# dmlc/difacto

Hardware: AMD Instinct MI355X
Metric: examples/sec (FM SGD worker step, Criteo-shape, V_dim=64) (higher is better)
Workload: dtype f32

## Files before the change

difacto_amd/csrc/dfh_api.hip:

```cpp
#include <algorithm>
#include <chrono>
#include <cstring>
#include <mutex>
#include <new>
#include <thread>

#include <hip/hip_ext.h>
#include <rocprim/rocprim.hpp>

#include "dfh_kernels.hip"
#include "dfh_localize.hip"
#include "dfh_update.hip"
#include "dfh_riders.hip"

using namespace dfh;

namespace dfh {
static thread_local std::string g_err;
void set_error(const std::string& msg) { g_err = msg; }
}

struct dfh_ctx {
  int device = 0;
  hipStream_t stream = nullptr;
// ... 2424 lines not shown
  }
  DFH_ARG(total == nrows, "dfh_batch_gather_rows: the segments must hold nrows rows");
  DFH_HIP(hipSetDevice(b->ctx->device));
  phase_begin(b);
  rc = prep_begin(b);
  if (rc) return rc;
  hipStream_t s = prep_of(b);
  b->d_raw = b->o_raw; b->d_offset = b->o_offset; b->d_value = b->o_value; b->d_label = b->o_label;
  const size_t o_off = 0, o_lab = (b->max_rows + 1) * 4, o_idx = ((o_lab + b->max_rows * 4 + 255) & ~(size_t)255),
               o_val = o_idx + b->max_nnz * 8, stage_total = o_val + b->max_nnz * 4;
  (void)stage_total;
  rc = ensure_stage(b, o_idx + (b->max_rows + 1) * 4);
  if (rc) return rc;
  if (b->staged_pending) {
    if (hipEventQuery(b->ev_staged) != hipSuccess) DFH_HIP(hipEventSynchronize(b->ev_staged));
    b->staged_pending = false;
  }
  memcpy(b->h_stage + o_off, off32.data(), (nrows + 1) * 4);
  memcpy(b->h_stage + o_lab, label, nrows * 4);
  uint32_t* h_rows = reinterpret_cast<uint32_t*>(b->h_stage + o_idx);
  size_t at = 0;
  for (int g = 0; g < nseg; ++g) {
    for (size_t i = 0; i < seg_rows[g]; ++i) {
      DFH_ARG(rows[g][i] < bufs[g]->nrows, "dfh_batch_gather_rows: row number beyond the buffer");
      h_rows[at + i] = rows[g][i];
    }
    at += seg_rows[g];
  }
  uint32_t* d_rows = b->d_pos;
  DFH_HIP(hipMemcpyAsync(b->d_offset, b->h_stage + o_off, (nrows + 1) * 4, hipMemcpyHostToDevice, s));
  DFH_HIP(hipMemcpyAsync(b->d_label, b->h_stage + o_lab, nrows * 4, hipMemcpyHostToDevice, s));
  DFH_HIP(hipMemcpyAsync(d_rows, h_rows, nrows * 4, hipMemcpyHostToDevice, s));
  DFH_HIP(hipEventRecord(b->ev_staged, s));
  b->staged_pending = true;
  at = 0;
  for (int g = 0; g < nseg; ++g) {
    dfh_rowbuf* rb = bufs[g];
    if (seg_rows[g] == 0) continue;
    DFH_HIP(hipStreamWaitEvent(s, rb->ev_loaded, 0));
    const unsigned blocks = (unsigned)std::min<size_t>((seg_rows[g] + 3) / 4, 4096);
    hipLaunchKernelGGL(k_gather_rows, dim3(blocks), dim3(256), 0, s, rb->d_off, rb->d_idx, rb->has_value ? rb->d_val : (const float*)nullptr,
                       d_rows + at, (uint32_t)seg_rows[g], b->d_offset + at, b->d_raw, any_value ? b->d_value : (float*)nullptr);
    {
      std::lock_guard<std::mutex> lk(rb->mu);
      dfh_rowbuf::Used* u = nullptr;
      for (auto& x : rb->used)
        if (x.stream == s) u = &x;
      if (!u) {
        hipEvent_t ev = nullptr;
        DFH_HIP(hipEventCreateWithFlags(&ev, hipEventDisableTiming));
        rb->used.push_back({s, ev, false});
        u = &rb->used.back();
      }
      DFH_HIP(hipEventRecord(u->ev, s));
      u->pending = true;
    }
    at += seg_rows[g];
  }
  DFH_HIP(hipGetLastError());
  b->nrows = nrows;
  b->nnz = nnz;
  b->has_value = any_value;
  b->has_cnt = false;
  b->localized = false;
  b->looked_up = nullptr;
  return DFH_OK;
}

namespace {
__global__ void __launch_bounds__(256) k_gather_rows_staged(const uint32_t* __restrict__ src_off, const uint64_t* __restrict__ src_idx,
                                                            const float* __restrict__ src_val, const uint32_t* __restrict__ h_rows,
                                                            const uint32_t* __restrict__ h_off, const float* __restrict__ h_lab, uint32_t n,
                                                            uint32_t* __restrict__ dst_off, float* __restrict__ dst_lab,
                                                            uint64_t* __restrict__ dst_idx, float* __restrict__ dst_val, int write_end) {
  constexpr uint32_t GR = 32;
  __shared__ uint32_t s_lo[GR], s_len[GR], s_d0[GR];
  const uint32_t lane = threadIdx.x & 63u, w = threadIdx.x >> 6;
  for (uint32_t q0 = blockIdx.x * GR; q0 < n; q0 += gridDim.x * GR) {
    const uint32_t m = min(GR, n - q0);
    __syncthreads();
    if (threadIdx.x < m) {
      const uint32_t q = q0 + threadIdx.x;
      const uint32_t r = h_rows[q], o = h_off[q];
      const uint32_t lo = src_off[r];
      s_lo[threadIdx.x] = lo;
      s_len[threadIdx.x] = src_off[r + 1] - lo;
      s_d0[threadIdx.x] = o;
      dst_off[q] = o;
      dst_lab[q] = h_lab[q];
    }
    if (threadIdx.x == 255 && write_end && q0 + m == n) dst_off[n] = h_off[n];
    __syncthreads();
    for (uint32_t t = w; t < m; t += 4u) {
      const uint32_t lo = s_lo[t], len = s_len[t], d0 = s_d0[t];
      for (uint32_t j = lane; j < len; j += 64u) {
        dst_idx[d0 + j] = src_idx[lo + j];
        if (dst_val) dst_val[d0 + j] = src_val ? src_val[lo + j] : 1.0f;
      }
    }
  }
}
}

namespace {
int gather_queued(dfh_batch* b, hipStream_t s) {
  for (const auto& g : b->gsegs) {
    dfh_rowbuf* rb = g.rb;
    std::lock_guard<std::mutex> lk(rb->mu);
    dfh_rowbuf::Used* u = nullptr;
    for (auto& x : rb->used)
      if (x.stream == s) u = &x;
    if (!u) {
      hipEvent_t ev = nullptr;
      DFH_HIP(hipEventCreateWithFlags(&ev, hipEventDisableTiming));
      rb->used.push_back({s, ev, false});
      u = &rb->used.back();
    }
    DFH_HIP(hipEventRecord(u->ev, s));
    u->pending = true;
  }
  DFH_HIP(hipEventRecord(b->ev_staged, s));
  b->staged_pending = true;
  b->gather_pending = false;
  return DFH_OK;
}
int gather_alone(dfh_batch* b, hipStream_t s) {
  for (const auto& g : b->gsegs) {
    dfh_rowbuf* rb = g.rb;
    const unsigned blocks = (unsigned)std::min<size_t>((g.n + 31) / 32, 2048);
    hipLaunchKernelGGL(k_gather_rows_staged, dim3(blocks), dim3(256), 0, s, rb->d_off, rb->d_idx,
                       rb->has_value ? rb->d_val : (const float*)nullptr, b->g_rows + g.at, b->g_off + g.at, b->g_lab + g.at, (uint32_t)g.n,
                       b->d_offset + g.at, b->d_label + g.at, b->d_raw, b->gather_any_value ? b->d_value : (float*)nullptr,
                       g.at + g.n == b->nrows ? 1 : 0);
  }
  DFH_HIP(hipGetLastError());
  return gather_queued(b, s);
}
}

namespace {
void launch_loc_stage(dfh_batch* b, int stage, hipStream_t s, dfh_table* probe = nullptr) {
  const LocView& v = b->loc_v;
  switch (stage) {
    case RID_COUNT:
      if (b->loc_big) hipLaunchKernelGGL(k_loc_count<LOC_BIG_BUCKETS>, dim3(v.ntiles), dim3(LOC_TILE_THREADS), 0, s, v);
      else if (b->loc_fuse_gather) hipLaunchKernelGGL(k_loc_count_gather<LOC_MAX_BUCKETS>, dim3(v.ntiles), dim3(LOC_TILE_THREADS), 0, s, v, b->gsrc);
      else hipLaunchKernelGGL(k_loc_count<LOC_MAX_BUCKETS>, dim3(v.ntiles), dim3(LOC_TILE_THREADS), 0, s, v);
      break;
    case RID_SCATTER:
      if (b->loc_big) hipLaunchKernelGGL(k_loc_scatter<LOC_BIG_BUCKETS>, dim3(v.ntiles), dim3(LOC_TILE_THREADS), 0, s, v);
      else hipLaunchKernelGGL(k_loc_scatter<LOC_MAX_BUCKETS>, dim3(v.ntiles), dim3(LOC_TILE_THREADS), 0, s, v);
      break;
    case RID_SORT:
      hipLaunchKernelGGL(k_loc_sort, dim3(b->loc_gsort), dim3(LOC_SORT_THREADS), 0, s, v);
      break;
    default:
      if (probe) hipLaunchKernelGGL(k_loc_emit<true>, dim3(b->loc_gsort), dim3(LOC_EMIT_THREADS), 0, s, v, b->loc_o, probe->v, b->d_urow);
      else hipLaunchKernelGGL(k_loc_emit<false>, dim3(b->loc_gsort), dim3(LOC_EMIT_THREADS), 0, s, v, b->loc_o, TableView{}, (uint32_t*)nullptr);
      break;
  }
}

void pend_remove(dfh_ctx* c, dfh_batch* b) {
  auto it = std::find(c->pend.begin(), c->pend.end(), b);
  if (it != c->pend.end()) c->pend.erase(it);
}

int flush_pending(dfh_batch* b) {
  dfh_ctx* c = b->ctx;
  if (b->pend_stage >= RID_STAGES) return DFH_OK;
  {
    TimeScope ts(c, DFH_K_LOCALIZE);
    for (int st = b->pend_stage; st < RID_STAGES; ++st) launch_loc_stage(b, st, c->stream);
  }
  b->pend_stage = RID_STAGES;
  pend_remove(c, b);
  DFH_HIP(hipGetLastError());
  return DFH_OK;
}

void collect_riders(dfh_ctx* c, int slot, bool can_ride, uint32_t main_groups, RiderSet* rs) {
  rs->n = 0;
  rs->ngroups = 0;
  rs->period = 1;
  rs->start = 0;
  rs->first[0] = 0;
  if (!c->single_queue || c->pend.empty()) return;
  for (size_t i = 0; i < c->pend.size(); ++i) {
    dfh_batch* p = c->pend[i];
    while (p->pend_stage < RID_STAGES && c->rider_slot[p->pend_stage] == slot) {
      const int st = p->pend_stage;
      if (c->rider_alone[st] || !can_ride || rs->n == MAX_RIDERS) {
        TimeScope ts(c, DFH_K_LOCALIZE);
        launch_loc_stage(p, st, c->stream);
        ++p->pend_stage;
        continue;
      }
      Rider& r = rs->r[rs->n];
      r.v = p->loc_v;
      r.o = p->loc_o;
      r.kind = (uint32_t)st;
      r.nblk = (st == RID_COUNT || st == RID_SCATTER) ? (uint32_t)p->loc_v.ntiles : p->loc_gsort;
      rs->first[rs->n + 1] = rs->first[rs->n] + ((r.nblk + 7u) & ~7u);
      ++rs->n;
      ++p->pend_stage;
      break;
    }
  }
  for (uint32_t j = 1; j < rs->n; ++j) {
    if (rs->r[j].kind == RID_EMIT && rs->r[0].kind != RID_EMIT) {
      std::swap(rs->r[0], rs->r[j]);
      uint32_t at = 0;
      for (uint32_t q = 0; q < rs->n; ++q) {
        rs->first[q] = at;
        at += (rs->r[q].nblk + 7u) & ~7u;
      }
      rs->first[rs->n] = at;
      break;
    }
  }
  c->pend.erase(std::remove_if(c->pend.begin(), c->pend.end(), [](dfh_batch* p) { return p->pend_stage >= RID_STAGES; }), c->pend.end());
  rs->ngroups = rs->first[rs->n] / 8u;
  for (uint32_t q = rs->n + 1; q <= (uint32_t)MAX_RIDERS; ++q) rs->first[q] = rs->first[rs->n];
  if (rs->ngroups) {
    rs->start = (uint32_t)((uint64_t)main_groups * (uint64_t)c->rider_start[slot] / 100u);
    const uint32_t left = main_groups - rs->start;
    uint32_t per = (uint32_t)std::max(1, c->rider_period[slot]);
    if (rs->ngroups > 1) per = std::min(per, (left + rs->ngroups - 1u) / (rs->ngroups - 1u));
    rs->period = std::max(1u, per);
  }
}

int localize_impl(dfh_batch* b, uint64_t max_index, dfh_table* probe) {
  dfh_ctx* c = b->ctx;
  DFH_HIP(hipSetDevice(c->device));
  const uint32_t N = (uint32_t)b->nnz;
  if (probe && N) {
    if (int rcr = table_reserve(probe, N)) return rcr;
  }
  {
    int rc = prep_begin(b);
    if (rc) return rc;
  }
  hipStream_t s = prep_of(b);
  b->looked_up = nullptr;
  if (b->pend_stage < RID_STAGES) {
    int rc = flush_pending(b);
    if (rc) return rc;
  }
  if (N == 0) {
    if (b->gather_pending) {
      int rcg = gather_alone(b, s);
      if (rcg) return rcg;
    }
    DFH_HIP(hipMemsetAsync(b->d_U, 0, 64 * sizeof(uint32_t), s));
    DFH_HIP(hipMemsetAsync(b->d_col_ptr, 0, 4, s));
    b->seg_nb = 0;
    b->localized = true;
    return prep_end(b);
  }
  const int g = grid_for_threads(N, c);
  TimeScope* tsp = new TimeScope(c, DFH_K_LOCALIZE, s);
  int P = 0;
  bool cold = true;
  if (b->spl_P > 0 && N / (uint32_t)b->spl_P >= (uint32_t)LOC_MIN_AVG && N / (uint32_t)b->spl_P <= (uint32_t)LOC_MAX_AVG) {
    P = b->spl_P;
    cold = false;
  } else {
#ifndef DFH_LOC_SMALL_AVG
#define DFH_LOC_SMALL_AVG 192
#endif
    const size_t avg_bucket = N <= 65536u ? (size_t)DFH_LOC_SMALL_AVG : (size_t)LOC_AVG_BUCKET;
    const size_t P_want = (N + avg_bucket - 1) / avg_bucket;
    if (P_want <= (size_t)LOC_MAX_BUCKETS) P = (int)std::max<size_t>(1, P_want);
    else if (N / LOC_MAX_BUCKETS <= (uint32_t)LOC_MAX_AVG) P = LOC_MAX_BUCKETS;
    else if (P_want <= (size_t)LOC_BIG_BUCKETS) P = (int)P_want;
    else if (N / LOC_BIG_BUCKETS <= (uint32_t)LOC_MAX_AVG) P = LOC_BIG_BUCKETS;
  }
  b->loc_fuse_gather = b->gather_pending && b->gather_fusable && !cold && P > 0 && P <= LOC_MAX_BUCKETS && !b->force_radix &&
                       !c->single_queue && !getenv("DFH_GATHER_ALONE");
  if (b->gather_pending && !b->loc_fuse_gather) {
    int rcg = gather_alone(b, s);
    if (rcg) return rcg;
  }
  if (P > 0 && !b->force_radix) {
    LocView& v = b->loc_v;
    v.raw = b->d_raw;
    v.n = N;
    v.max_index = max_index;
    v.P = P;
    const bool big = P > LOC_MAX_BUCKETS;
    v.bstride = big ? LOC_BIG_BUCKETS : LOC_MAX_BUCKETS;
    v.ntiles = (int)((N + LOC_TILE - 1) / LOC_TILE);
    v.force_global = b->force_sort_fallback ? 1 : 0;
    v.tb = N > 1 ? std::min(16, __builtin_clz(N - 1)) : 16;
    v.nrows = (uint32_t)b->nrows;
    v.offset = b->d_offset;
    v.rowid = b->d_pos;
    v.smp_key = b->d_smp_key;
    v.smp_pos = b->d_smp_pos;
    v.smp_rank = b->d_smp_rank;
    v.spl_key = b->d_spl_key;
    v.spl_pos = b->d_spl_pos;
    v.packed = b->d_packed;
    v.run_off = b->d_run_off;
    v.btotal = b->d_btotal;
    v.bstart = b->d_bstart;
// ... 653 lines not shown
```

difacto_amd/csrc/dfh_localize.hip:

```cpp
#ifndef DFH_LOCALIZE_HIP_
#define DFH_LOCALIZE_HIP_
#include "dfh_internal.h"

namespace dfh {

constexpr int LOC_OVERSAMPLE = 8;
constexpr int LOC_MAX_BUCKETS = 1024;
constexpr int LOC_BIG_BUCKETS = 4096;
constexpr int LOC_AVG_BUCKET = 384;
constexpr int LOC_MIN_AVG = 48;
constexpr int LOC_MAX_AVG = 700;
constexpr int LOC_LDS_CAP = 1024;
#ifndef DFH_LOC_TILE
#define DFH_LOC_TILE 2048
#endif
#ifndef DFH_LOC_TILE_THREADS
#define DFH_LOC_TILE_THREADS 1024
#endif
constexpr int LOC_TILE = DFH_LOC_TILE;
constexpr int LOC_TILE_THREADS = DFH_LOC_TILE_THREADS;
constexpr int LOC_PER_THREAD = LOC_TILE / LOC_TILE_THREADS;
constexpr int LOC_SORT_THREADS = 256;
constexpr int LOC_EMIT_THREADS = 256;

struct LocView {
  const uint64_t* raw;
  uint32_t n;
  uint64_t max_index;
  int P;
  int bstride;
  int ntiles;
  int force_global;
  int tb;
  uint32_t nrows;
  const uint32_t* offset;
  const uint32_t* rowid;
  uint64_t* smp_key;
  uint32_t* smp_pos;
  uint32_t* smp_rank;
  uint64_t* spl_key;
  uint32_t* spl_pos;
  uint32_t* packed;
  uint32_t* run_off;
  uint32_t* btotal;
  uint32_t* bstart;
  uint64_t* bkeys;
  uint32_t* bpos;
  uint64_t* skeys;
  uint32_t* spos;
  uint64_t* first_key;
  uint64_t* last_key;
  uint32_t* nheads;
  uint32_t* lh;
  uint32_t* split_n;
};

struct SegListsOut {
  uint2* mid;
  SegEnt* mid_ent;
  uint2* hot;
  SegEnt* hot_ent;
  uint2* few;
  SegEnt* few_ent;
};

__device__ __forceinline__ uint64_t make_key(uint64_t id, uint64_t max_index) {
  const uint64_t m = (max_index == ~0ULL) ? (id == ~0ULL ? 0ULL : id) : id % max_index;
  return reverse_bytes(m);
}

constexpr int LOC_XCDS = 8;

__device__ __forceinline__ bool comp_less(uint64_t ka, uint32_t pa, uint64_t kb, uint32_t pb) {
  return ka < kb || (ka == kb && pa < pb);
}

template <int NWAVES>
__device__ __forceinline__ uint32_t block_exclusive_scan(uint32_t val, uint32_t* wsum , uint32_t* total) {
  uint32_t s = val;
#pragma unroll
  for (int o = 1; o < 64; o <<= 1) {
    const uint32_t y = __shfl_up(s, o, 64);
    if ((int)(threadIdx.x & 63) >= o) s += y;
  }
  __syncthreads();
  if ((threadIdx.x & 63) == 63) wsum[threadIdx.x >> 6] = s;
  __syncthreads();
  uint32_t woff = 0, tot = 0;
#pragma unroll
  for (int w = 0; w < NWAVES; ++w) {
    const uint32_t x = wsum[w];
    if (w < (int)(threadIdx.x >> 6)) woff += x;
    tot += x;
  }
  if (total) *total = tot;
  return woff + s - val;
}

template <int NWAVES>
__device__ __forceinline__ uint32_t block_exclusive_max(uint32_t val, uint32_t* wmax , uint32_t* total) {
  uint32_t s = val;
#pragma unroll
  for (int o = 1; o < 64; o <<= 1) {
    const uint32_t y = __shfl_up(s, o, 64);
    if ((int)(threadIdx.x & 63) >= o) s = max(s, y);
  }
  __syncthreads();
  if ((threadIdx.x & 63) == 63) wmax[threadIdx.x >> 6] = s;
  __syncthreads();
  uint32_t before = 0, tot = 0;
#pragma unroll
  for (int w = 0; w < NWAVES; ++w) {
    const uint32_t x = wmax[w];
    if (w < (int)(threadIdx.x >> 6)) before = max(before, x);
    tot = max(tot, x);
  }
  if (total) *total = tot;
  uint32_t prev = __shfl_up(s, 1, 64);
  if ((threadIdx.x & 63) == 0) prev = 0;
  return max(before, prev);
}

__device__ __forceinline__ uint32_t ss_sample_pos(uint32_t t, uint32_t stride, uint32_t n) {
  const uint32_t j = (uint32_t)(splitmix64(t) >> 33) % stride;
  return min(t * stride + j, n - 1);
}

__global__ void __launch_bounds__(256) k_ss_sample(LocView v) {
  const uint32_t S = (uint32_t)v.P * LOC_OVERSAMPLE;
  const uint32_t stride = max(1u, v.n / S);
  for (uint32_t t = blockIdx.x * blockDim.x + threadIdx.x; t < S; t += gridDim.x * blockDim.x) {
    const uint32_t i = ss_sample_pos(t, stride, v.n);
    v.smp_key[t] = make_key(v.raw[i], v.max_index);
    v.smp_pos[t] = i << v.tb;
    v.smp_rank[t] = 0;
  }
}

__global__ void __launch_bounds__(256) k_ss_rank(LocView v) {
  __shared__ uint64_t ck[256];
  __shared__ uint32_t cp[256];
  const uint32_t S = (uint32_t)v.P * LOC_OVERSAMPLE;
  const uint32_t ntile = (S + 255) / 256;
  const uint32_t ti = blockIdx.x / ntile, tj = blockIdx.x % ntile;
  const uint32_t col = tj * 256 + threadIdx.x;
  ck[threadIdx.x] = col < S ? v.smp_key[col] : ~0ULL;
  cp[threadIdx.x] = col < S ? v.smp_pos[col] : ~0u;
  const uint32_t row = ti * 256 + threadIdx.x;
  const uint64_t mk = row < S ? v.smp_key[row] : 0;
  const uint32_t mp = row < S ? v.smp_pos[row] : 0;
  __syncthreads();
  const uint32_t lim = min(256u, S - tj * 256);
  uint32_t rank = 0;
#pragma unroll 8
  for (uint32_t j = 0; j < lim; ++j) {
    const bool less = comp_less(ck[j], cp[j], mk, mp) || (ck[j] == mk && cp[j] == mp && tj * 256 + j < row);
    rank += less ? 1u : 0u;
  }
  if (row < S && rank) atomicAdd(&v.smp_rank[row], rank);
}

__global__ void __launch_bounds__(256) k_loc_splitters(LocView v) {
  const uint32_t S = (uint32_t)v.P * LOC_OVERSAMPLE;
  for (uint32_t t = blockIdx.x * blockDim.x + threadIdx.x; t < S; t += gridDim.x * blockDim.x) {
    const uint32_t r = v.smp_rank[t];
    if (r > 0 && r % LOC_OVERSAMPLE == 0) {
      v.spl_key[r / LOC_OVERSAMPLE - 1] = v.smp_key[t];
      v.spl_pos[r / LOC_OVERSAMPLE - 1] = v.smp_pos[t];
    }
  }
}

constexpr int LOC_GATHER_ROWS = 1024;
constexpr int LOC_GATHER_SEGS = 4;
struct GatherSrc {
  int nseg;
  uint32_t seg_row0[LOC_GATHER_SEGS + 1];
  const uint32_t* src_off[LOC_GATHER_SEGS];
  const uint64_t* src_idx[LOC_GATHER_SEGS];
  const float* src_val[LOC_GATHER_SEGS];
  const uint32_t* h_rows;
  const uint32_t* h_off;
  const float* h_lab;
  const uint32_t* h_tile_row;
  uint64_t* dst_raw;
  float* dst_val;
  uint32_t* dst_off;
  float* dst_lab;
};
constexpr size_t loc_gather_smem() { return (size_t)(LOC_GATHER_ROWS + 1) * 4 + 4 + (size_t)LOC_GATHER_ROWS * 8; }
template <typename T>
__device__ __forceinline__ T loc_sel(const T (&a)[LOC_GATHER_SEGS], uint32_t sg) {
  T r = a[0];
#pragma unroll
  for (int x = 1; x < LOC_GATHER_SEGS; ++x) r = sg == (uint32_t)x ? a[x] : r;
  return r;
}

template <int MAXB>
constexpr size_t loc_count_smem() { return (size_t)MAXB * 16; }
template <int MAXB, int THREADS>
constexpr size_t loc_scatter_smem() { return (size_t)MAXB * 4 + (THREADS / 64) * 4; }
constexpr size_t loc_sort_smem() { return (size_t)LOC_LDS_CAP * 24 + 2 * (LOC_SORT_THREADS / 64) * 4; }
constexpr size_t loc_emit_smem() { return (2 * (LOC_EMIT_THREADS / 64) + 4) * 4; }

template <int MAXB, int THREADS, bool GATHER = false>
__device__ __forceinline__ void loc_count_block(const LocView& v, const uint32_t bid, const uint32_t nblk, char* smem,
                                                const GatherSrc* gp = nullptr) {
  constexpr int PER = LOC_TILE / THREADS;
  static_assert(PER * THREADS == LOC_TILE, "a tile is a whole number of elements per thread");
  uint64_t* sk = reinterpret_cast<uint64_t*>(smem);
  uint32_t* sp = reinterpret_cast<uint32_t*>(smem + (size_t)MAXB * 8);
  uint32_t* hist = sp + MAXB;
  const int P = v.P;
  for (int b = threadIdx.x; b < P; b += THREADS) {
    hist[b] = 0;
    sk[b] = b < P - 1 ? v.spl_key[b] : ~0ULL;
    sp[b] = b < P - 1 ? v.spl_pos[b] : ~0u;
  }
  const uint32_t base = bid * LOC_TILE;
  if (bid == 0 && threadIdx.x == 0 && v.split_n) *v.split_n = 0u;
  uint64_t key[PER];
  if (GATHER) {
    const GatherSrc& g = *gp;
    uint32_t* roff = reinterpret_cast<uint32_t*>(smem + loc_count_smem<MAXB>());
    uint64_t* rsrc = reinterpret_cast<uint64_t*>(roff + LOC_GATHER_ROWS + 2);
    const uint32_t row0 = g.h_tile_row[bid], row1 = g.h_tile_row[bid + 1];
    const uint32_t nr = min(row1, v.nrows - 1u) - row0 + 1u;
    for (uint32_t q = threadIdx.x; q <= nr; q += THREADS) roff[q] = g.h_off[row0 + q];
    for (uint32_t q = threadIdx.x; q < nr; q += THREADS) {
      const uint32_t r = row0 + q;
      uint32_t sg = 0;
#pragma unroll
      for (int x = 1; x < LOC_GATHER_SEGS; ++x) sg += (x < g.nseg && r >= g.seg_row0[x]) ? 1u : 0u;
      rsrc[q] = ((uint64_t)loc_sel(g.src_off, sg)[g.h_rows[r]] << 2) | sg;
    }
    __syncthreads();
#pragma unroll
    for (int e = 0; e < PER; ++e) {
      const uint32_t i = base + e * THREADS + threadIdx.x;
      key[e] = ~0ULL;
      if (i < v.n) {
        uint32_t lo = 0, hi = nr - 1u;
        while (lo < hi) {
          const uint32_t mid = (lo + hi + 1u) >> 1;
          if (roff[mid] <= i) lo = mid; else hi = mid - 1u;
        }
        const uint64_t sw = rsrc[lo];
        const uint32_t sg = (uint32_t)(sw & 3u);
        const size_t at = (size_t)(sw >> 2) + (i - roff[lo]);
        const uint64_t id = loc_sel(g.src_idx, sg)[at];
        g.dst_raw[i] = id;
        if (g.dst_val) {
          const float* sv = loc_sel(g.src_val, sg);
          g.dst_val[i] = sv ? sv[at] : 1.0f;
        }
        key[e] = make_key(id, v.max_index);
      }
    }
  } else {
#pragma unroll
    for (int e = 0; e < PER; ++e) {
      const uint32_t i = base + e * THREADS + threadIdx.x;
      key[e] = i < v.n ? make_key(v.raw[i], v.max_index) : ~0ULL;
    }
  }
  {
    uint32_t* __restrict__ rowid = const_cast<uint32_t*>(v.rowid);
    const uint32_t* __restrict__ offset = GATHER ? gp->h_off : v.offset;
    const uint32_t rpb = (v.nrows + nblk - 1) / nblk;
    const uint32_t r0 = bid * rpb, r1 = min(v.nrows, r0 + rpb);
    for (uint32_t r = r0 + threadIdx.x; r < r1; r += THREADS) {
      const uint32_t b0 = offset[r], e = offset[r + 1];
      if (GATHER) {
        gp->dst_off[r] = b0;
        gp->dst_lab[r] = gp->h_lab[r];
        if (r + 1 == v.nrows) gp->dst_off[r + 1] = e;
      }
      for (uint32_t j = b0; j < e; ++j) rowid[j] = r;
    }
  }
  __syncthreads();
  int lo[PER], hi[PER];
#pragma unroll
  for (int e = 0; e < PER; ++e) { lo[e] = 0; hi[e] = P - 1; }
  for (int step = P; step > 1; step = (step + 1) >> 1) {
#pragma unroll
    for (int e = 0; e < PER; ++e) {
      if (lo[e] < hi[e]) {
        const uint32_t i = base + e * THREADS + threadIdx.x;
        const int mid = (lo[e] + hi[e]) >> 1;
        if (comp_less(key[e], i << v.tb, sk[mid], sp[mid])) hi[e] = mid; else lo[e] = mid + 1;
      }
    }
  }
#pragma unroll
  for (int e = 0; e < PER; ++e) {
    const uint32_t i = base + e * THREADS + threadIdx.x;
    if (i < v.n) {
      const uint32_t r = atomicAdd(&hist[lo[e]], 1u);
      v.packed[i] = ((uint32_t)lo[e] << 16) | r;
    }
  }
  __syncthreads();
  for (int b = threadIdx.x; b < P; b += THREADS) {
    const uint32_t h = hist[b];
    v.run_off[bid * P + b] = h ? atomicAdd(&v.btotal[(bid & (LOC_XCDS - 1)) * MAXB + b], h) : 0u;
  }
}

template <int MAXB>
__global__ void __launch_bounds__(LOC_TILE_THREADS) k_loc_count(LocView v) {
  __shared__ __attribute__((aligned(16))) char smem[loc_count_smem<MAXB>()];
  loc_count_block<MAXB, LOC_TILE_THREADS>(v, blockIdx.x, gridDim.x, smem);
}
template <int MAXB>
__global__ void __launch_bounds__(LOC_TILE_THREADS) k_loc_count_gather(LocView v, GatherSrc g) {
  __shared__ __attribute__((aligned(16))) char smem[loc_count_smem<MAXB>() + loc_gather_smem()];
  loc_count_block<MAXB, LOC_TILE_THREADS, true>(v, blockIdx.x, gridDim.x, smem, &g);
}


template <int MAXB, int THREADS>
__device__ __forceinline__ void loc_scatter_block(const LocView& v, const uint32_t bid, char* smem) {
  constexpr int PER = LOC_TILE / THREADS;
  constexpr int LOC_BPT = MAXB / THREADS;
  static_assert(LOC_BPT * THREADS == MAXB, "the scan of the bucket totals gives every thread the same number of buckets");
  uint32_t* off = reinterpret_cast<uint32_t*>(smem);
  uint32_t* wsum = off + MAXB;
  const int P = v.P;
  const uint32_t xcd = bid & (LOC_XCDS - 1);
  const uint32_t base = bid * LOC_TILE;
  uint64_t raw[PER];
  uint32_t pk[PER], rw[PER];
#pragma unroll
  for (int e = 0; e < PER; ++e) {
    const uint32_t i = min(base + e * THREADS + threadIdx.x, v.n - 1);
    raw[e] = v.raw[i];
    pk[e] = v.packed[i];
    rw[e] = v.rowid[i];
  }
  const int b0 = threadIdx.x * LOC_BPT;
  uint32_t tt[LOC_BPT], ro[LOC_BPT];
  uint32_t sum = 0;
#pragma unroll
  for (int q = 0; q < LOC_BPT; ++q) {
    const int bb = min(b0 + q, P - 1);
    const uint32_t in = b0 + q < P ? 1u : 0u;
    tt[q] = 0;
    ro[q] = v.run_off[bid * P + bb];
#pragma unroll
    for (int x = 0; x < LOC_XCDS; ++x) {
      const uint32_t h = v.btotal[x * MAXB + bb];
      tt[q] += h;
      ro[q] += (x < (int)xcd ? 1u : 0u) * h;
    }
    tt[q] *= in;
    ro[q] *= in;
    sum += tt[q];
  }
  uint32_t total;
  uint32_t ex = block_exclusive_scan<THREADS / 64>(sum, wsum, &total);
#pragma unroll
  for (int q = 0; q < LOC_BPT; ++q) {
    if (b0 + q < P) {
      off[b0 + q] = ex + ro[q];
      if (bid == 0) v.bstart[b0 + q] = ex;
    }
    ex += tt[q];
  }
  if (bid == 0 && threadIdx.x == 0) v.bstart[P] = total;
  __syncthreads();
#pragma unroll
  for (int e = 0; e < PER; ++e) {
    const uint32_t i = base + e * THREADS + threadIdx.x;
    if (i < v.n) {
      const uint32_t dst = off[pk[e] >> 16] + (pk[e] & 0xFFFFu);
      v.bkeys[dst] = make_key(raw[e], v.max_index);
      v.bpos[dst] = (i << v.tb) | (rw[e] & ((1u << v.tb) - 1u));
    }
  }
}

template <int MAXB>
__global__ void __launch_bounds__(LOC_TILE_THREADS) k_loc_scatter(LocView v) {
  __shared__ __attribute__((aligned(16))) char smem[loc_scatter_smem<MAXB, LOC_TILE_THREADS>()];
  loc_scatter_block<MAXB, LOC_TILE_THREADS>(v, blockIdx.x, smem);
}

__device__ __forceinline__ bool loc_sort_bucket(const LocView& v, uint32_t beg, uint32_t n, uint64_t* ak, uint32_t* ap,
                                                uint64_t* bk, uint32_t* bp, const uint64_t** sk_out, const uint32_t** sp_out) {
  const uint64_t* gk = v.bkeys + beg;
  const uint32_t* gp = v.bpos + beg;
  const bool in_lds = n <= LOC_LDS_CAP && !v.force_global;
  uint64_t* sk = bk;
  uint32_t* sp = bp;
  if (in_lds) {
    const uint32_t lane = threadIdx.x & 63;
    for (uint32_t c0 = (threadIdx.x >> 6) * 64; c0 < n; c0 += LOC_SORT_THREADS) {
      const uint32_t idx = c0 + lane;
      const bool valid = idx < n;
      const uint64_t mk = valid ? gk[idx] : ~0ULL;
      const uint32_t mp = valid ? gp[idx] : ~0u;
      const int klo = (int)(uint32_t)mk, khi = (int)(uint32_t)(mk >> 32);
      uint32_t rank = 0;
#pragma unroll 8
      for (int j = 0; j < 64; ++j) {
        const uint64_t ok = ((uint64_t)(uint32_t)__builtin_amdgcn_readlane(khi, j) << 32) | (uint32_t)__builtin_amdgcn_readlane(klo, j);
        const uint32_t op = (uint32_t)__builtin_amdgcn_readlane((int)mp, j);
        rank += comp_less(ok, op, mk, mp) ? 1u : 0u;
      }
      if (valid) {
        bk[c0 + rank] = mk;
        bp[c0 + rank] = mp;
      }
    }
    __syncthreads();
    constexpr int E = LOC_LDS_CAP / LOC_SORT_THREADS;
    static_assert(E * LOC_SORT_THREADS == LOC_LDS_CAP && LOC_SORT_THREADS % 64 == 0, "a thread carries E elements of a full bucket");
    uint64_t* dk = ak;
    uint32_t* dp = ap;
    uint32_t sh = 6;
    for (uint32_t L = 64; L < n; L <<= 1, ++sh) {
      uint64_t mk[E];
      uint32_t mp[E], cnt[E], sb[E], len[E];
#pragma unroll
      for (int e = 0; e < E; ++e) {
        const uint32_t idx = threadIdx.x + e * LOC_SORT_THREADS;
        const bool valid = idx < n;
        len[e] = 0;
        cnt[e] = 0;
        if (e * LOC_SORT_THREADS >= n) continue;
        mk[e] = valid ? sk[idx] : 0ULL;
        mp[e] = valid ? sp[idx] : 0u;
        const uint32_t sib = ((idx >> sh) ^ 1u) << sh;
        sb[e] = min(sib, n);
        len[e] = valid ? min(sib + L, n) - sb[e] : 0u;
        cnt[e] = 0;
      }
      for (uint32_t step = L; step; step >>= 1) {
        uint64_t ok[E];
        uint32_t op[E];
#pragma unroll
        for (int e = 0; e < E; ++e) {
          if (e * LOC_SORT_THREADS >= n) continue;
          const uint32_t t = cnt[e] + step;
          const uint32_t at = t <= len[e] ? sb[e] + t - 1u : 0u;
          ok[e] = sk[at];
          op[e] = sp[at];
        }
#pragma unroll
        for (int e = 0; e < E; ++e) {
          if (e * LOC_SORT_THREADS >= n) continue;
          const uint32_t t = cnt[e] + step;
          if (t <= len[e] && comp_less(ok[e], op[e], mk[e], mp[e])) cnt[e] = t;
        }
      }
#pragma unroll
      for (int e = 0; e < E; ++e) {
        const uint32_t idx = threadIdx.x + e * LOC_SORT_THREADS;
        if (idx < n) {
          const uint32_t r = idx >> sh;
          const uint32_t dst = ((r & ~1u) << sh) + (idx - (r << sh)) + cnt[e];
          dk[dst] = mk[e];
          dp[dst] = mp[e];
        }
      }
      __syncthreads();
      uint64_t* tk = sk; sk = dk; dk = tk;
      uint32_t* tp = sp; sp = dp; dp = tp;
    }
    *sk_out = sk;
    *sp_out = sp;
  } else {
    uint64_t* xk = v.bkeys + beg;
    uint32_t* xp = v.bpos + beg;
    uint64_t* yk = v.skeys + beg;
    uint32_t* yp = v.spos + beg;
    const uint32_t lane = threadIdx.x & 63;
    for (uint32_t c0 = (threadIdx.x >> 6) * 64; c0 < n; c0 += LOC_SORT_THREADS) {
      const uint32_t idx = c0 + lane;
      const bool valid = idx < n;
      const uint64_t mk = valid ? xk[idx] : ~0ULL;
      const uint32_t mp = valid ? xp[idx] : ~0u;
      const uint32_t lim = min(64u, n - c0);
      uint32_t rank = 0;
      for (uint32_t j = 0; j < lim; ++j) rank += comp_less(xk[c0 + j], xp[c0 + j], mk, mp) ? 1u : 0u;
      if (valid) {
        yk[c0 + rank] = mk;
        yp[c0 + rank] = mp;
      }
    }
    __syncthreads();
    uint64_t* srck = yk; uint32_t* srcp = yp;
    uint64_t* dstk = xk; uint32_t* dstp = xp;
    for (uint32_t L = 64; L < n; L <<= 1) {
      for (uint32_t idx = threadIdx.x; idx < n; idx += blockDim.x) {
        const uint64_t mk = srck[idx];
        const uint32_t mp = srcp[idx];
        const uint32_t r = idx / L;
        const uint32_t pair_base = (r & ~1u) * L;
        const uint32_t sib = (r ^ 1u) * L;
        uint32_t lo = min(sib, n), hi = min(sib + L, n);
        const uint32_t sib_beg = lo;
        while (lo < hi) {
          const uint32_t mid = (lo + hi) >> 1;
          if (comp_less(srck[mid], srcp[mid], mk, mp)) lo = mid + 1; else hi = mid;
        }
        const uint32_t dst = pair_base + (idx - r * L) + (lo - sib_beg);
        dstk[dst] = mk;
        dstp[dst] = mp;
      }
      __syncthreads();
      uint64_t* tk = srck; srck = dstk; dstk = tk;
      uint32_t* tp = srcp; srcp = dstp; dstp = tp;
    }
    if (srck != yk) {
      for (uint32_t t = threadIdx.x; t < n; t += blockDim.x) {
        yk[t] = srck[t];
        yp[t] = srcp[t];
      }
    }
    __syncthreads();
  }
  if (!in_lds) {
    *sk_out = v.skeys + beg;
    *sp_out = v.spos + beg;
  }
  return in_lds;
}

struct BucketSummary {
  uint32_t nheads, lh;
  uint64_t first_key, last_key;
};
__device__ __forceinline__ BucketSummary loc_bucket_summary(const uint64_t* sk, uint32_t n, uint32_t (*red)[LOC_SORT_THREADS / 64]) {
  uint32_t cnt = 0, last = 0;
  for (uint32_t t = 1 + threadIdx.x; t < n; t += blockDim.x) {
    if (sk[t] != sk[t - 1]) {
      ++cnt;
      last = t;
    }
  }
#pragma unroll
  for (int o = 32; o > 0; o >>= 1) {
    cnt += __shfl_xor(cnt, o, 64);
    last = max(last, (uint32_t)__shfl_xor(last, o, 64));
  }
  if ((threadIdx.x & 63) == 0) {
    red[0][threadIdx.x >> 6] = cnt;
    red[1][threadIdx.x >> 6] = last;
  }
  __syncthreads();
  BucketSummary r;
  r.nheads = 1;
  r.lh = 0;
  r.first_key = 0;
  r.last_key = 0;
  if (threadIdx.x == 0) {
    for (int w = 0; w < LOC_SORT_THREADS / 64; ++w) {
      r.nheads += red[0][w];
      r.lh = max(r.lh, red[1][w]);
    }
    r.first_key = sk[0];
    r.last_key = sk[n - 1];
  }
  return r;
}

__device__ __forceinline__ void loc_sort_block(const LocView& v, const uint32_t bid, const uint32_t nblk, char* smem) {
  uint64_t* ak = reinterpret_cast<uint64_t*>(smem);
  uint64_t* bk = ak + LOC_LDS_CAP;
  uint32_t* ap = reinterpret_cast<uint32_t*>(bk + LOC_LDS_CAP);
  uint32_t* bp = ap + LOC_LDS_CAP;
  uint32_t (*red)[LOC_SORT_THREADS / 64] = reinterpret_cast<uint32_t (*)[LOC_SORT_THREADS / 64]>(bp + LOC_LDS_CAP);
  for (uint32_t b = bid; b < (uint32_t)v.P; b += nblk) {
    __syncthreads();
    const uint32_t beg = v.bstart[b], end = v.bstart[b + 1];
    const uint32_t n = end - beg;
    if (threadIdx.x < LOC_XCDS) v.btotal[threadIdx.x * v.bstride + b] = 0;
    if (n == 0) {
      if (threadIdx.x == 0) {
        v.nheads[b] = 0;
        v.lh[b] = 0;
        v.first_key[b] = 0;
        v.last_key[b] = 0;
      }
      continue;
    }
    const uint64_t* sk;
    const uint32_t* sp;
    if (loc_sort_bucket(v, beg, n, ak, ap, bk, bp, &sk, &sp)) {
      for (uint32_t t = threadIdx.x; t < n; t += LOC_SORT_THREADS) {
        v.skeys[beg + t] = sk[t];
        v.spos[beg + t] = sp[t];
      }
    }
    const BucketSummary sm = loc_bucket_summary(sk, n, red);
    if (threadIdx.x == 0) {
      v.nheads[b] = sm.nheads;
      v.lh[b] = sm.lh;
      v.first_key[b] = sm.first_key;
      v.last_key[b] = sm.last_key;
    }
  }
}
__global__ void __launch_bounds__(LOC_SORT_THREADS) k_loc_sort(LocView v) {
  __shared__ __attribute__((aligned(16))) char smem[loc_sort_smem()];
  loc_sort_block(v, blockIdx.x, gridDim.x, smem);
}

template <int NW, bool PROBE>
__device__ __forceinline__ void loc_emit_bucket(const LocView& v, uint32_t b, uint32_t beg, uint32_t n, const uint64_t* sk,
                                                const uint32_t* sp, uint32_t cont, uint32_t ubase, uint32_t carry1,
                                                const float* __restrict__ value,
                                                uint64_t* __restrict__ feaids, uint32_t* __restrict__ col_ptr,
                                                uint32_t* __restrict__ index, uint32_t* __restrict__ s_row,
                                                float* __restrict__ s_val, uint32_t* __restrict__ d_U, const SegListsOut& sl,
                                                uint32_t* wsum, uint32_t* wmax, uint32_t* n_mid, uint32_t* n_hot,
                                                uint32_t* n_few, const TableView& tab, uint32_t* __restrict__ urow) {
  const uint32_t P = (uint32_t)v.P;
  const uint32_t moff = beg / (BWD_SMALL + 1) + 2 * b, hoff = beg / (BWD_MID + 1) + 2 * b, foff = beg / 2 + 2 * b;
  uint32_t run_heads = 0, run_max1 = carry1;
  for (uint32_t base = 0; base < n; base += blockDim.x) {
    const uint32_t t = base + threadIdx.x;
    const uint32_t i = beg + t;
    const bool valid = t < n;
    uint64_t key = 0;
    uint32_t tag = 0;
    bool head = false;
    if (valid) {
      key = sk[t];
      tag = sp[t];
      head = t == 0 ? !cont : key != sk[t - 1];
    }
    const uint32_t pos = tag >> v.tb;
    uint32_t nh, mx;
    const uint32_t ex = block_exclusive_scan<NW>(head ? 1u : 0u, wsum, &nh);
    const uint32_t pm = block_exclusive_max<NW>(head ? i + 1 : 0u, wmax, &mx);
    if (valid) {
      const uint32_t incl = run_heads + ex + (head ? 1u : 0u);
      const uint32_t uid = ubase + incl - 1;
      const uint32_t prev1 = max(run_max1, pm);
      if (head) {
        feaids[uid] = key;
        col_ptr[uid] = i;
        if (PROBE) urow[uid] = find_or_insert(tab, key);
        if (prev1) {
          const uint32_t len = i - (prev1 - 1);
          const SegEnt e = make_uint4(uid - 1, prev1 - 1, i, 0u);
          if (len > BWD_MID) sl.hot_ent[hoff + atomicAdd(n_hot, 1u)] = e;
          else if (len > BWD_SMALL) sl.mid_ent[moff + atomicAdd(n_mid, 1u)] = e;
          else if (len > 1) sl.few_ent[foff + atomicAdd(n_few, 1u)] = e;
        }
      }
      index[pos] = uid;
      uint32_t row = tag & ((1u << v.tb) - 1u);
      {
        const uint32_t step = 1u << v.tb;
        uint32_t lo = 0, hi = v.nrows > row ? (v.nrows - 1u - row) >> v.tb : 0u;
        while (lo < hi) {
          const uint32_t mid = (lo + hi + 1u) >> 1;
          if (v.offset[row + mid * step] <= pos) lo = mid; else hi = mid - 1u;
        }
        row += lo * step;
      }
      s_row[i] = row;
      if (value) s_val[i] = value[pos];
      if (i == v.n - 1) {
        *d_U = uid + 1;
        col_ptr[uid + 1] = v.n;
        const uint32_t lbeg = head ? i : prev1 - 1, len = v.n - lbeg;
        const SegEnt e = make_uint4(uid, lbeg, v.n, 0u);
        if (len > BWD_MID) sl.hot_ent[hoff + atomicAdd(n_hot, 1u)] = e;
        else if (len > BWD_SMALL) sl.mid_ent[moff + atomicAdd(n_mid, 1u)] = e;
        else if (len > 1) sl.few_ent[foff + atomicAdd(n_few, 1u)] = e;
      }
      if (P > 1) {
        const uint64_t m = ((uint64_t)i * P + v.n - 1) / v.n;
        if (m >= 1 && m <= P - 1 && (m * v.n) / P == i) {
          v.spl_key[m - 1] = key;
          v.spl_pos[m - 1] = tag;
        }
      }
    }
    run_heads += nh;
    run_max1 = max(run_max1, mx);
  }
  __syncthreads();
  if (threadIdx.x == 0) {
    sl.mid[b] = make_uint2(*n_mid, moff);
    sl.hot[b] = make_uint2(*n_hot, hoff);
    sl.few[b] = make_uint2(*n_few, foff);
  }
}

struct EmitOut {
  const float* value;
  uint64_t* feaids;
  uint32_t* col_ptr;
  uint32_t* index;
  uint32_t* s_row;
  float* s_val;
  uint32_t* d_U;
  SegListsOut sl;
};

template <bool PROBE>
__device__ __forceinline__ void loc_emit_block(const LocView& v, const EmitOut& o, const TableView& tab, uint32_t* __restrict__ urow,
                                               const uint32_t bid, const uint32_t nblk, char* smem) {
  constexpr int NW = LOC_EMIT_THREADS / 64;
  uint32_t* wsum = reinterpret_cast<uint32_t*>(smem);
  uint32_t* wmax = wsum + NW;
  uint32_t& sh_cont = wmax[NW];
  uint32_t& n_mid = wmax[NW + 1];
  uint32_t& n_hot = wmax[NW + 2];
  uint32_t& n_few = wmax[NW + 3];
  const SegListsOut& sl = o.sl;
  const uint32_t P = (uint32_t)v.P;
  for (uint32_t b = bid; b < P; b += nblk) {
    __syncthreads();
    const uint32_t beg = v.bstart[b], end = v.bstart[b + 1];
    const uint32_t n = end - beg;
    if (threadIdx.x == 0) {
      n_mid = 0;
      n_hot = 0;
      n_few = 0;
      if (n == 0) {
        sl.mid[b] = make_uint2(0u, 0u);
        sl.hot[b] = make_uint2(0u, 0u);
        sl.few[b] = make_uint2(0u, 0u);
      }
    }
    if (n == 0) continue;
    uint32_t part = 0, carry1 = 0;
    for (uint32_t q0 = threadIdx.x; q0 <= b; q0 += LOC_EMIT_THREADS) {
      const uint32_t bq = v.bstart[q0], nq = v.bstart[q0 + 1] - bq;
      if (nq == 0) continue;
      int p = (int)q0 - 1;
      while (p >= 0 && v.bstart[p + 1] == v.bstart[p]) --p;
      const uint32_t c = (p >= 0 && v.first_key[q0] == v.last_key[p]) ? 1u : 0u;
      if (q0 == b) {
        sh_cont = c;
      } else {
        part += v.nheads[q0] - c;
        const uint32_t l = v.lh[q0];
        if (l > 0) carry1 = max(carry1, bq + l + 1);
        else if (!c) carry1 = max(carry1, bq + 1);
      }
    }
    uint32_t ubase, carry_all;
    block_exclusive_scan<NW>(part, wsum, &ubase);
    block_exclusive_max<NW>(carry1, wmax, &carry_all);
    __syncthreads();
    loc_emit_bucket<NW, PROBE>(v, b, beg, n, v.skeys + beg, v.spos + beg, sh_cont, ubase, carry_all, o.value, o.feaids, o.col_ptr,
                               o.index, o.s_row, o.s_val, o.d_U, sl, wsum, wmax, &n_mid, &n_hot, &n_few, tab, urow);
  }
}

template <bool PROBE>
__global__ void __launch_bounds__(LOC_EMIT_THREADS) k_loc_emit(LocView v, EmitOut o, TableView tab, uint32_t* __restrict__ urow) {
  __shared__ __attribute__((aligned(16))) char smem[loc_emit_smem()];
  loc_emit_block<PROBE>(v, o, tab, urow, blockIdx.x, gridDim.x, smem);
}

}
#endif
```

Measured before the change: 82.32 million.

## Use DPP wave scans, restructure bucket merge sort, and hoist splitter emission

Replaces the shuffle-based block scans and reductions with DPP-based wave-inclusive scans plus readlane. The bucket-offset scan in the scatter kernel moves ahead of the element loads. The sort kernel now takes dynamic LDS and processes merge elements two at a time with fewer live registers, and a rank loop's unroll factor is lowered. Splitter key emission moves out of the per-element path into a small strided loop over only the splitter indices in each bucket. Together these aim to cut instruction count and register pressure in the localize stages, at the risk of subtle indexing bugs in the new merge destination and splitter math.

```diff
diff --git a/difacto_amd/csrc/dfh_api.hip b/difacto_amd/csrc/dfh_api.hip
--- a/difacto_amd/csrc/dfh_api.hip
+++ b/difacto_amd/csrc/dfh_api.hip
@@ -2600,7 +2600,7 @@
       else hipLaunchKernelGGL(k_loc_scatter<LOC_MAX_BUCKETS>, dim3(v.ntiles), dim3(LOC_TILE_THREADS), 0, s, v);
       break;
     case RID_SORT:
-      hipLaunchKernelGGL(k_loc_sort, dim3(b->loc_gsort), dim3(LOC_SORT_THREADS), 0, s, v);
+      hipLaunchKernelGGL(k_loc_sort, dim3(b->loc_gsort), dim3(LOC_SORT_THREADS), loc_sort_smem(), s, v);
       break;
     default:
       if (probe) hipLaunchKernelGGL(k_loc_emit<true>, dim3(b->loc_gsort), dim3(LOC_EMIT_THREADS), 0, s, v, b->loc_o, probe->v, b->d_urow);
diff --git a/difacto_amd/csrc/dfh_localize.hip b/difacto_amd/csrc/dfh_localize.hip
--- a/difacto_amd/csrc/dfh_localize.hip
+++ b/difacto_amd/csrc/dfh_localize.hip
@@ -75,50 +75,45 @@
   return ka < kb || (ka == kb && pa < pb);
 }
 
+template <bool MAX>
+__device__ __forceinline__ uint32_t wave_inclusive(uint32_t x) {
+#define DFH_DPP_STEP(ctrl, row_mask)                                                                      \
+  {                                                                                                       \
+    const uint32_t y = (uint32_t)__builtin_amdgcn_update_dpp(0, (int)x, ctrl, row_mask, 0xf, false);    \
+    x = MAX ? max(x, y) : x + y;                                                                          \
+  }
+  DFH_DPP_STEP(0x111, 0xf)
+  DFH_DPP_STEP(0x112, 0xf)
+  DFH_DPP_STEP(0x114, 0xf)
+  DFH_DPP_STEP(0x118, 0xf)
+  DFH_DPP_STEP(0x142, 0xa)
+  DFH_DPP_STEP(0x143, 0xc)
+#undef DFH_DPP_STEP
+  return x;
+}
+
+template <bool MAX, int NWAVES>
+__device__ __forceinline__ uint32_t block_exclusive(uint32_t val, uint32_t* wtot , uint32_t* total) {
+  static_assert(NWAVES <= 64, "one lane per wave");
+  const int lane = (int)(threadIdx.x & 63);
+  const int w = __builtin_amdgcn_readfirstlane((int)(threadIdx.x >> 6));
+  const uint32_t s = wave_inclusive<MAX>(val);
+  __syncthreads();
+  if (lane == 63) wtot[w] = s;
+  __syncthreads();
+  const uint32_t x = wave_inclusive<MAX>(lane < NWAVES ? wtot[lane] : 0u);
+  const uint32_t before = w ? (uint32_t)__builtin_amdgcn_readlane((int)x, w - 1) : 0u;
+  if (total) *total = (uint32_t)__builtin_amdgcn_readlane((int)x, NWAVES - 1);
+  const uint32_t prev = (uint32_t)__builtin_amdgcn_update_dpp(0, (int)s, 0x138, 0xf, 0xf, false);
+  return MAX ? max(before, prev) : before + prev;
+}
 template <int NWAVES>
 __device__ __forceinline__ uint32_t block_exclusive_scan(uint32_t val, uint32_t* wsum , uint32_t* total) {
-  uint32_t s = val;
-#pragma unroll
-  for (int o = 1; o < 64; o <<= 1) {
-    const uint32_t y = __shfl_up(s, o, 64);
-    if ((int)(threadIdx.x & 63) >= o) s += y;
-  }
-  __syncthreads();
-  if ((threadIdx.x & 63) == 63) wsum[threadIdx.x >> 6] = s;
-  __syncthreads();
-  uint32_t woff = 0, tot = 0;
-#pragma unroll
-  for (int w = 0; w < NWAVES; ++w) {
-    const uint32_t x = wsum[w];
-    if (w < (int)(threadIdx.x >> 6)) woff += x;
-    tot += x;
-  }
-  if (total) *total = tot;
-  return woff + s - val;
-}
-
+  return block_exclusive<false, NWAVES>(val, wsum, total);
+}
 template <int NWAVES>
 __device__ __forceinline__ uint32_t block_exclusive_max(uint32_t val, uint32_t* wmax , uint32_t* total) {
-  uint32_t s = val;
-#pragma unroll
-  for (int o = 1; o < 64; o <<= 1) {
-    const uint32_t y = __shfl_up(s, o, 64);
-    if ((int)(threadIdx.x & 63) >= o) s = max(s, y);
-  }
-  __syncthreads();
-  if ((threadIdx.x & 63) == 63) wmax[threadIdx.x >> 6] = s;
-  __syncthreads();
-  uint32_t before = 0, tot = 0;
-#pragma unroll
-  for (int w = 0; w < NWAVES; ++w) {
-    const uint32_t x = wmax[w];
-    if (w < (int)(threadIdx.x >> 6)) before = max(before, x);
-    tot = max(tot, x);
-  }
-  if (total) *total = tot;
-  uint32_t prev = __shfl_up(s, 1, 64);
-  if ((threadIdx.x & 63) == 0) prev = 0;
-  return max(before, prev);
+  return block_exclusive<true, NWAVES>(val, wmax, total);
 }
 
 __device__ __forceinline__ uint32_t ss_sample_pos(uint32_t t, uint32_t stride, uint32_t n) {
@@ -331,6 +326,36 @@
   const int P = v.P;
   const uint32_t xcd = bid & (LOC_XCDS - 1);
   const uint32_t base = bid * LOC_TILE;
+  const int b0 = threadIdx.x * LOC_BPT;
+  uint32_t tt[LOC_BPT], ro[LOC_BPT];
+  uint32_t sum = 0;
+#pragma unroll
+  for (int q = 0; q < LOC_BPT; ++q) {
+    const int bb = min(b0 + q, P - 1);
+    const uint32_t in = b0 + q < P ? 1u : 0u;
+    tt[q] = 0;
+    ro[q] = v.run_off[bid * P + bb];
+#pragma unroll
+    for (int x = 0; x < LOC_XCDS; ++x) {
+      const uint32_t h = v.btotal[x * MAXB + bb];
+      tt[q] += h;
+      ro[q] += (x < (int)xcd ? 1u : 0u) * h;
+    }
+    tt[q] *= in;
+    ro[q] *= in;
+    sum += tt[q];
+  }
+  uint32_t total;
+  uint32_t ex = block_exclusive_scan<THREADS / 64>(sum, wsum, &total);
+#pragma unroll
+  for (int q = 0; q < LOC_BPT; ++q) {
+    if (b0 + q < P) {
+      off[b0 + q] = ex + ro[q];
+      if (bid == 0) v.bstart[b0 + q] = ex;
+    }
+    ex += tt[q];
+  }
+  if (bid == 0 && threadIdx.x == 0) v.bstart[P] = total;
   uint64_t raw[PER];
   uint32_t pk[PER], rw[PER];
 #pragma unroll
@@ -340,36 +365,6 @@
     pk[e] = v.packed[i];
     rw[e] = v.rowid[i];
   }
-  const int b0 = threadIdx.x * LOC_BPT;
-  uint32_t tt[LOC_BPT], ro[LOC_BPT];
-  uint32_t sum = 0;
-#pragma unroll
-  for (int q = 0; q < LOC_BPT; ++q) {
-    const int bb = min(b0 + q, P - 1);
-    const uint32_t in = b0 + q < P ? 1u : 0u;
-    tt[q] = 0;
-    ro[q] = v.run_off[bid * P + bb];
-#pragma unroll
-    for (int x = 0; x < LOC_XCDS; ++x) {
-      const uint32_t h = v.btotal[x * MAXB + bb];
-      tt[q] += h;
-      ro[q] += (x < (int)xcd ? 1u : 0u) * h;
-    }
-    tt[q] *= in;
-    ro[q] *= in;
-    sum += tt[q];
-  }
-  uint32_t total;
-  uint32_t ex = block_exclusive_scan<THREADS / 64>(sum, wsum, &total);
-#pragma unroll
-  for (int q = 0; q < LOC_BPT; ++q) {
-    if (b0 + q < P) {
-      off[b0 + q] = ex + ro[q];
-      if (bid == 0) v.bstart[b0 + q] = ex;
-    }
-    ex += tt[q];
-  }
-  if (bid == 0 && threadIdx.x == 0) v.bstart[P] = total;
   __syncthreads();
 #pragma unroll
   for (int e = 0; e < PER; ++e) {
@@ -404,7 +399,7 @@
       const uint32_t mp = valid ? gp[idx] : ~0u;
       const int klo = (int)(uint32_t)mk, khi = (int)(uint32_t)(mk >> 32);
       uint32_t rank = 0;
-#pragma unroll 8
+#pragma unroll 4
       for (int j = 0; j < 64; ++j) {
         const uint64_t ok = ((uint64_t)(uint32_t)__builtin_amdgcn_readlane(khi, j) << 32) | (uint32_t)__builtin_amdgcn_readlane(klo, j);
         const uint32_t op = (uint32_t)__builtin_amdgcn_readlane((int)mp, j);
@@ -417,53 +412,47 @@
     }
     __syncthreads();
     constexpr int E = LOC_LDS_CAP / LOC_SORT_THREADS;
-    static_assert(E * LOC_SORT_THREADS == LOC_LDS_CAP && LOC_SORT_THREADS % 64 == 0, "a thread carries E elements of a full bucket");
+    constexpr int G = 2;
+    static_assert(E * LOC_SORT_THREADS == LOC_LDS_CAP && E % G == 0 && LOC_SORT_THREADS % 64 == 0,
+                  "a thread carries E elements of a full bucket, G at a time");
     uint64_t* dk = ak;
     uint32_t* dp = ap;
     uint32_t sh = 6;
     for (uint32_t L = 64; L < n; L <<= 1, ++sh) {
-      uint64_t mk[E];
-      uint32_t mp[E], cnt[E], sb[E], len[E];
-#pragma unroll
-      for (int e = 0; e < E; ++e) {
-        const uint32_t idx = threadIdx.x + e * LOC_SORT_THREADS;
-        const bool valid = idx < n;
-        len[e] = 0;
-        cnt[e] = 0;
-        if (e * LOC_SORT_THREADS >= n) continue;
-        mk[e] = valid ? sk[idx] : 0ULL;
-        mp[e] = valid ? sp[idx] : 0u;
-        const uint32_t sib = ((idx >> sh) ^ 1u) << sh;
-        sb[e] = min(sib, n);
-        len[e] = valid ? min(sib + L, n) - sb[e] : 0u;
-        cnt[e] = 0;
-      }
-      for (uint32_t step = L; step; step >>= 1) {
-        uint64_t ok[E];
-        uint32_t op[E];
-#pragma unroll
-        for (int e = 0; e < E; ++e) {
-          if (e * LOC_SORT_THREADS >= n) continue;
-          const uint32_t t = cnt[e] + step;
-          const uint32_t at = t <= len[e] ? sb[e] + t - 1u : 0u;
-          ok[e] = sk[at];
-          op[e] = sp[at];
+      for (int g = 0; g < E && g * LOC_SORT_THREADS < (int)n; g += G) {
+        uint64_t mk[G];
+        uint32_t mp[G], at[G], end[G];
+#pragma unroll
+        for (int e = 0; e < G; ++e) {
+          const uint32_t idx = threadIdx.x + (g + e) * LOC_SORT_THREADS;
+          const bool valid = idx < n;
+          const uint32_t sib = ((idx >> sh) ^ 1u) << sh;
+          mk[e] = valid ? sk[idx] : 0ULL;
+          mp[e] = valid ? sp[idx] : 0u;
+          at[e] = min(sib, n);
+          end[e] = valid ? min(sib + L, n) : at[e];
         }
-#pragma unroll
-        for (int e = 0; e < E; ++e) {
-          if (e * LOC_SORT_THREADS >= n) continue;
-          const uint32_t t = cnt[e] + step;
-          if (t <= len[e] && comp_less(ok[e], op[e], mk[e], mp[e])) cnt[e] = t;
+        for (uint32_t step = L; step; step >>= 1) {
+          uint64_t ok[G];
+          uint32_t op[G];
+#pragma unroll
+          for (int e = 0; e < G; ++e) {
+            const uint32_t q = at[e] + step <= end[e] ? at[e] + step - 1u : 0u;
+            ok[e] = sk[q];
+            op[e] = sp[q];
+          }
+#pragma unroll
+          for (int e = 0; e < G; ++e)
+            if (at[e] + step <= end[e] && comp_less(ok[e], op[e], mk[e], mp[e])) at[e] += step;
         }
-      }
-#pragma unroll
-      for (int e = 0; e < E; ++e) {
-        const uint32_t idx = threadIdx.x + e * LOC_SORT_THREADS;
-        if (idx < n) {
-          const uint32_t r = idx >> sh;
-          const uint32_t dst = ((r & ~1u) << sh) + (idx - (r << sh)) + cnt[e];
-          dk[dst] = mk[e];
-          dp[dst] = mp[e];
+#pragma unroll
+        for (int e = 0; e < G; ++e) {
+          const uint32_t idx = threadIdx.x + (g + e) * LOC_SORT_THREADS;
+          if (idx < n) {
+            const uint32_t dst = idx + at[e] - min((idx & ~(L - 1u)) | L, n);
+            dk[dst] = mk[e];
+            dp[dst] = mp[e];
+          }
         }
       }
       __syncthreads();
@@ -542,11 +531,8 @@
       last = t;
     }
   }
-#pragma unroll
-  for (int o = 32; o > 0; o >>= 1) {
-    cnt += __shfl_xor(cnt, o, 64);
-    last = max(last, (uint32_t)__shfl_xor(last, o, 64));
-  }
+  cnt = (uint32_t)__builtin_amdgcn_readlane((int)wave_inclusive<false>(cnt), 63);
+  last = (uint32_t)__builtin_amdgcn_readlane((int)wave_inclusive<true>(last), 63);
   if ((threadIdx.x & 63) == 0) {
     red[0][threadIdx.x >> 6] = cnt;
     red[1][threadIdx.x >> 6] = last;
@@ -606,7 +592,7 @@
   }
 }
 __global__ void __launch_bounds__(LOC_SORT_THREADS) k_loc_sort(LocView v) {
-  __shared__ __attribute__((aligned(16))) char smem[loc_sort_smem()];
+  extern __shared__ __attribute__((aligned(16))) char smem[];
   loc_sort_block(v, blockIdx.x, gridDim.x, smem);
 }
 
@@ -676,16 +662,22 @@
         else if (len > BWD_SMALL) sl.mid_ent[moff + atomicAdd(n_mid, 1u)] = e;
         else if (len > 1) sl.few_ent[foff + atomicAdd(n_few, 1u)] = e;
       }
-      if (P > 1) {
-        const uint64_t m = ((uint64_t)i * P + v.n - 1) / v.n;
-        if (m >= 1 && m <= P - 1 && (m * v.n) / P == i) {
-          v.spl_key[m - 1] = key;
-          v.spl_pos[m - 1] = tag;
-        }
-      }
     }
     run_heads += nh;
     run_max1 = max(run_max1, mx);
+  }
+  if (P > 1) {
+    const uint64_t N = v.n;
+    const uint64_t m0 = max((uint64_t)beg * P / N + ((uint64_t)beg * P % N ? 1u : 0u), (uint64_t)1);
+    const uint64_t e1 = (uint64_t)(beg + n) * P;
+    const uint64_t m1 = min(e1 / N + (e1 % N ? 1u : 0u), (uint64_t)P);
+    for (uint64_t m = m0 + threadIdx.x; m < m1; m += blockDim.x) {
+      const uint32_t i = (uint32_t)(m * N / P);
+      if ((i * (uint64_t)P + N - 1) / N == m) {
+        v.spl_key[m - 1] = sk[i - beg];
+        v.spl_pos[m - 1] = sp[i - beg];
+      }
+    }
   }
   __syncthreads();
   if (threadIdx.x == 0) {
```

New measurement: 85.55 million (median of 6 runs). +3.9%, better.
